# StructuralNeurobiologyLab/SyConn

Measured on AMD Instinct MI355X. Metric: segmented Mvoxels/s (whole node), 128^3 EM tiles, higher is better.
Workload: dtype bf16; 1 GPU; BASELINE configs[1]: semseg_spine 3D U-Net on 128^3 uint8 tiles, 96 tiles per GPU per step in launch sets of 8 (sd_forward_labels_batch), random-init weights, HOST TO HOST: pinned host uint8 tiles -> H2D -> kernels -> pinned host uint8 labels (stored by the last kernel, no copy), 3 HIP streams, 2 buffer sets; tiles_per_launch_set=8, parallelism=tile-sharded x1, hip_streams_per_gpu=3, collective=none

## Files before the change

### syconn_amd/csrc/sd_kernels.hip

```cpp
#include "sd_internal.h"
#include "../../include/syconn_dense.h"
#include <algorithm>
#include <cstdlib>
#include <mutex>
#include <string>
#include <type_traits>
#include <utility>

#include "sd_device.h"

#include "sd_conv_mfma.h"


template <typename T, int KZ, typename IN, bool SPLIT = false>
__global__ __launch_bounds__(256) void k_conv_first(const FirstParams p) {
    constexpr int BZ = sd_bz(KZ), BY = sd_by(KZ), BX = SD_BX;
    constexpr int PZ = KZ / 2;
    constexpr int HZ = BZ + KZ - 1, HY = BY + 2, HX = BX + 2;
    constexpr int NH = HZ * HY * HX;
    constexpr int NTAP = KZ * 9;
    constexpr int NSTEP = (NTAP + 1) / 2;
    __shared__ float patch[NH];

    const int tid = threadIdx.x, lane = tid & 63, wave = tid >> 6;
// ... 153 lines not shown
            for (int e = 0; e < 4; ++e) acc[0][j][4 * q + e] = acc[1][j][4 * q + e] = bs[e];
        }

    __shared__ __attribute__((aligned(16))) float gtab[GN ? 2 * 1024 : 4];
    const float* gss = nullptr;
    if constexpr (GN) {
        const float* const g = reinterpret_cast<const float*>(reinterpret_cast<const char*>(p.gn) + blockIdx.z * p.tstride);
        for (int i = tid; i < 2 * p.Cs; i += 256) gtab[i] = g[i];
        __syncthreads();
        gss = gtab;
    }
    for (int c = 0; c < p.nchunk; ++c) {
        v8 xf[2], wf[2];
#pragma unroll
        for (int i = 0; i < 2; ++i) {
            v8 val = {};
            if (mv[i]) {
                const int sc = (SPLIT && c >= p.nchunk / 3) ? c - p.nchunk / 3 : c;
                val = *reinterpret_cast<const v8*>(src + ((size_t)sc * p.Ps + upconv_src_index(p, m[i])) * SD_CHUNK + (lane >> 5) * 8);
                if constexpr (GN) val = gn_apply8<T>(val, gss + c * SD_CHUNK + (lane >> 5) * 8, gss + p.Cs + c * SD_CHUNK + (lane >> 5) * 8, p.gn_relu);
            }
            xf[i] = val;
        }
#pragma unroll
        for (int j = 0; j < 2; ++j) wf[j] = *reinterpret_cast<const v8*>(wp + ((size_t)(c * 2 + j) * 64 + lane) * 8);
#pragma unroll
        for (int i = 0; i < 2; ++i)
#pragma unroll
            for (int j = 0; j < 2; ++j) acc[i][j] = Act<T>::mfma(wf[j], xf[i], acc[i][j]);
    }

    T* const dst = reinterpret_cast<T*>(reinterpret_cast<char*>(p.dst) + blockIdx.z * p.tstride);
    StoreGuard<T> sguard;
    const int H2 = p.Hd, W2 = p.Wd;
    const int half = lane >> 5;
#pragma unroll
    for (int i = 0; i < 2; ++i) {
        const unsigned mu = mv[i] ? (unsigned)m[i] : 0u;
        const unsigned xy = mu % (unsigned)(p.W * p.H), z = mu / (unsigned)(p.W * p.H), y = xy / (unsigned)p.W, x = xy - y * (unsigned)p.W;
#pragma unroll
        for (int j = 0; j < 2; ++j) {
            const int nbase = (nb * 2 + j) * 32;
#pragma unroll
            for (int qp = 0; qp < 2; ++qp) {
                unsigned d[2][2], dl[2][2];
#pragma unroll
                for (int h = 0; h < 2; ++h) {
                    const int q = 2 * qp + h;
                    float v[4];
#pragma unroll
                    for (int e = 0; e < 4; ++e) {
                        v[e] = acc[i][j][4 * q + e];
                        if constexpr (SPLIT) v[e] *= p.oscale;
                        if (p.relu) v[e] = fmaxf(v[e], 0.f);
                    }
                    if constexpr (SPLIT) {
                        split_pk(v[0], v[1], d[h][0], dl[h][0]);
                        split_pk(v[2], v[3], d[h][1], dl[h][1]);
                    } else {
                        d[h][0] = Act<T>::pack2(v[0], v[1]);
                        d[h][1] = Act<T>::pack2(v[2], v[3]);
                    }
                    sguard.see_signed(d[h][0]); sguard.see_signed(d[h][1]);
                }
                swap32(d[0][0], d[1][0]);
                swap32(d[0][1], d[1][1]);
                if constexpr (SPLIT) { swap32(dl[0][0], dl[1][0]); swap32(dl[0][1], dl[1][1]); }
                const int n8 = nbase + 8 * (2 * qp + half);
                if (mv[i] && n8 < p.ntot) {
                    const int tap = n8 / p.Cd, co = n8 - tap * p.Cd;
                    const int a = (p.kz == 2) ? (tap >> 2) : 0, b = (tap >> 1) & 1, cx = tap & 1;
                    const size_t vo = ((size_t)(z * p.kz + a) * H2 + (2 * y + b)) * W2 + (2 * x + cx);
                    typedef __attribute__((ext_vector_type(4))) unsigned u4;
                    *reinterpret_cast<u4*>(dst + ((size_t)(co >> 4) * p.Pd + vo) * SD_CHUNK + (co & 15)) = u4{d[0][0], d[0][1], d[1][0], d[1][1]};
                    if constexpr (SPLIT)
                        *reinterpret_cast<u4*>(dst + ((size_t)((co + p.Cd) >> 4) * p.Pd + vo) * SD_CHUNK + (co & 15)) = u4{dl[0][0], dl[0][1], dl[1][0], dl[1][1]};
                }
            }
        }
    }
    sguard.flush(p.ovf);
}

template <typename T, int NCH, int NTAB, bool WL, bool GN, bool SPLIT = false, int G = 1>
__global__ __launch_bounds__(256) void k_upconv_rows(const UpconvParams p) {
    constexpr int NX = SPLIT ? 2 * NCH : NCH;
    constexpr int NV = SPLIT ? 3 * NCH : NCH;
    static_assert(!(SPLIT && GN), "split plan: no deferred GroupNorm");
    static_assert(G == 1 || (WL && NTAB % (2 * G) == 0), "channel groups: LDS weights, whole tiles of each x-tap per group");
    using v8 = typename Act<T>::v8;
    using v4 = typename Act<T>::v4;
    typedef __attribute__((ext_vector_type(4))) unsigned u4;
    constexpr int CDR = NTAB * 16;
    constexpr int NTL = NTAB / G;
    constexpr int TPT = NTL / 2;
    constexpr int CD = NTL * 16;
    constexpr int ROW = 4 * CD;
    constexpr int PPV = ROW / 16;
    constexpr int SWM = (PPV % 8 == 0) ? 7 : (PPV % 4 == 0) ? 3 : (PPV % 2 == 0) ? 1 : 0;
    extern __shared__ __attribute__((aligned(16))) char smem[];
    const int tid = threadIdx.x, lane = tid & 63, wave = tid >> 6, half = lane >> 5, vl = lane & 31;
    char* const tile = smem + wave * (32 * ROW);
    const long M = (long)p.D * p.H * p.W;
    const T* const src = reinterpret_cast<const T*>(reinterpret_cast<const char*>(p.src) + blockIdx.z * p.tstride);
    const T* const wp = reinterpret_cast<const T*>(p.wpack);
    char* const dst = reinterpret_cast<char*>(p.dst) + blockIdx.z * p.tstride;
    const int H2 = p.Hd, W2 = p.Wd;
    StoreGuard<T> sguard;
    __shared__ __attribute__((aligned(16))) float gtab[GN ? 2 * NCH * SD_CHUNK : 4];
    const float* gss = nullptr;
    if constexpr (GN) {
        const float* const g = reinterpret_cast<const float*>(reinterpret_cast<const char*>(p.gn) + blockIdx.z * p.tstride);
        for (int i = tid; i < 2 * NCH * SD_CHUNK; i += 256) gtab[i] = g[i];
        __syncthreads();
        gss = gtab;
    }

    const char* const wlds = smem + 4 * 32 * ROW;
    const int a_wg = WL ? (int)blockIdx.y / G : 0;
    const int grp = G > 1 ? (int)blockIdx.y % G : 0;
    auto tile_of = [&](int ab, int jl) { return G == 1 ? ab * NTAB + jl : ab * NTAB + (jl / TPT) * (NTAB / 2) + grp * TPT + jl % TPT; };
    if constexpr (WL && G > 1) {
        for (int i = tid; i < NTL * NV * 64; i += 256) {
            const int piece = i >> 6, jl = piece / NV, c = piece - jl * NV, tl = tile_of(a_wg, jl);
            *reinterpret_cast<u4*>(smem + 4 * 32 * ROW + (size_t)i * 16) =
                *reinterpret_cast<const u4*>(reinterpret_cast<const char*>(wp) + ((((size_t)(tl >> 1) * NV + c) * 2 + (tl & 1)) * 64 + (i & 63)) * 16);
        }
        __syncthreads();
    } else if constexpr (WL) {
        const int first_blk = (a_wg * NTAB) >> 1, last_blk = (a_wg * NTAB + NTAB - 1) >> 1;
        const int nbytes = (last_blk - first_blk + 1) * NV * 2048;
        const char* const wsrc = reinterpret_cast<const char*>(wp) + (size_t)first_blk * NV * 2048;
        for (int o = tid * 16; o < nbytes; o += 256 * 16)
            *reinterpret_cast<u4*>(smem + 4 * 32 * ROW + o) = *reinterpret_cast<const u4*>(wsrc + o);
        __syncthreads();
    }
    for (long m0 = ((long)blockIdx.x * 4 + wave) * 32; m0 < M; m0 += WL ? (long)gridDim.x * 128 : M) {
    const long m = m0 + vl;
    const bool mv = m < M;
    const size_t sidx = mv ? upconv_src_index(p, m) : 0;
    v8 xf[NX];
#pragma unroll
    for (int c = 0; c < NX; ++c) {
        v8 val = {};
        if (mv) val = *reinterpret_cast<const v8*>(src + ((size_t)c * p.Ps + sidx) * SD_CHUNK + half * 8);
        xf[c] = val;
    }
    if constexpr (GN) {
#pragma unroll
        for (int c = 0; c < NCH; ++c) {
            if (mv) xf[c] = gn_apply8<T>(xf[c], gss + c * SD_CHUNK + half * 8, gss + p.Cs + c * SD_CHUNK + half * 8, p.gn_relu);
            asm volatile("" ::: "memory");
        }
    }
    const int ab0 = WL ? a_wg : 0, nab = WL ? ab0 + 1 : p.kz * 2;
#pragma unroll 1
    for (int ab = ab0; ab < nab; ++ab) {
        f32x16 acc[NTL];
#pragma unroll
        for (int j = 0; j < NTL; ++j)
#pragma unroll
            for (int q = 0; q < 4; ++q) {
                const f32x4 b = *reinterpret_cast<const f32x4*>(p.bias + 32 * tile_of(ab, j) + 8 * q + 4 * half);
#pragma unroll
                for (int e = 0; e < 4; ++e) acc[j][4 * q + e] = b[e];
            }
#pragma unroll
        for (int c = 0; c < NV; ++c) {
#pragma unroll
            for (int j = 0; j < NTL; ++j) {
                const int tl = ab * NTAB + j;
                v8 wf;
                if constexpr (WL && G > 1) {
                    wf = *reinterpret_cast<const v8*>(wlds + (((j * NV + c) * 64 + lane) * 16));
                } else if constexpr (WL) {
                    const int tloc = ab * NTAB + j - 2 * ((ab0 * NTAB) >> 1);
                    wf = *reinterpret_cast<const v8*>(wlds + ((((tloc >> 1) * NV + c) * 2 + (tloc & 1)) * 64 + lane) * 16);
                } else {
                    wf = *reinterpret_cast<const v8*>(wp + ((((size_t)(tl >> 1) * NV + c) * 2 + (tl & 1)) * 64 + lane) * 8);
                }
                acc[j] = Act<T>::mfma(wf, xf[(SPLIT && c >= NCH) ? c - NCH : c], acc[j]);
            }
        }
#pragma unroll
        for (int pass = 0; pass < (SPLIT ? 2 : 1); ++pass) {
#pragma unroll
        for (int j = 0; j < NTL; ++j) {
#pragma unroll
            for (int q = 0; q < 4; ++q) {
                v4 o;
#pragma unroll
                for (int e = 0; e < 4; ++e) {
                    float v = acc[j][4 * q + e];
                    if constexpr (SPLIT) v *= p.oscale;
                    if (p.relu) v = fmaxf(v, 0.f);
                    if constexpr (SPLIT) {
                        const T h = (T)v;
                        o[e] = pass == 0 ? h : (T)(v - (float)h);
                    } else {
                        o[e] = (T)v;
                    }
                }
                if (pass == 0) {
                    typedef __attribute__((ext_vector_type(2))) unsigned u2g;
                    const u2g ob = __builtin_bit_cast(u2g, o);
                    sguard.see_signed(ob.x); sguard.see_signed(ob.y);
                }
                const int pc = (4 * j + q) ^ (vl & SWM);
                *reinterpret_cast<v4*>(tile + vl * ROW + pc * 16 + half * 8) = o;
            }
        }
        const int a = (p.kz == 2) ? (ab >> 1) : 0, b = ab & 1;
        size_t ovv[2];
        bool okv[2];
#pragma unroll
        for (int e = 0; e < 2; ++e) {
            const long mm = m0 + (lane >> 2) + 16 * e;
            okv[e] = mm < M;
            const unsigned mu = (unsigned)(okv[e] ? mm : 0), xy = mu % (unsigned)(p.W * p.H), z = mu / (unsigned)(p.W * p.H);
            const unsigned y = xy / (unsigned)p.W, x = xy - y * (unsigned)p.W;
            ovv[e] = ((size_t)(z * p.kz + a) * H2 + (2 * y + b)) * W2 + 2 * x;
        }
#pragma unroll
        for (int it = 0; it < (32 * PPV) / 64; ++it) {
            const int u = it * 64 + lane;
            const int chunk = u >> 7, r = u & 127;
            const int v = r >> 2, tap = (r >> 1) & 1, hf = r & 1;
            const int piece = tap * (CD / 8) + chunk * 2 + hf;
            if (okv[it & 1]) {
                const size_t ov = ovv[it & 1] + tap;
                const u4 val = *reinterpret_cast<const u4*>(tile + v * ROW + ((piece ^ (v & SWM)) * 16));
                *reinterpret_cast<u4*>(dst + (((size_t)(grp * (CD / 16) + chunk + pass * (CDR / 16)) * p.Pd + ov) * SD_CHUNK + hf * 8) * sizeof(T)) = val;
            }
        }
        }
    }
    }
    sguard.flush(p.ovf);
}

__device__ __forceinline__ void decode_zyx(unsigned v, unsigned W, unsigned H, int& x, int& y, int& z) {
    const unsigned r = v / W, zz = r / H;
    x = (int)(v - r * W); y = (int)(r - zz * H); z = (int)zz;
}
template <typename T>
__global__ __launch_bounds__(256) void k_maxpool(const PoolParams p) {
    using v8 = typename Act<T>::v8;
    const int ng = p.C / 8;
    const long total = (long)p.Do * p.Ho * p.Wo * ng;
    const T* const src = reinterpret_cast<const T*>(reinterpret_cast<const char*>(p.src) + blockIdx.z * p.tstride);
    T* const dst = reinterpret_cast<T*>(reinterpret_cast<char*>(p.dst) + blockIdx.z * p.tstride);
    const long npv = (long)p.Do * p.Ho * p.Wo;
    for (long idx = (long)blockIdx.x * 256 + threadIdx.x; idx < total; idx += (long)gridDim.x * 256) {
        const unsigned pv = (unsigned)(idx >> 1), ch = pv / (unsigned)npv;
        const long v = pv - ch * (unsigned)npv;
        const int cg = (int)ch * 2 + (int)(idx & 1);
        int xo, yo, zo;
        decode_zyx((unsigned)v, (unsigned)p.Wo, (unsigned)p.Ho, xo, yo, zo);
        float mx[8];
#pragma unroll
        for (int e = 0; e < 8; ++e) mx[e] = -INFINITY;
        for (int dz = 0; dz < p.kz; ++dz) {
            const int z = zo * p.kz + dz;
            if (z >= p.D) continue;
#pragma unroll
            for (int dy = 0; dy < 2; ++dy) {
                const int y = yo * 2 + dy;
                if (y >= p.H) continue;
#pragma unroll
                for (int dx = 0; dx < 2; ++dx) {
                    const int x = xo * 2 + dx;
                    if (x >= p.W) continue;
                    const v8 val = *reinterpret_cast<const v8*>(src + ((size_t)(cg >> 1) * p.Ps + ((size_t)z * p.H + y) * p.W + x) * SD_CHUNK + (cg & 1) * 8);
#pragma unroll
                    for (int e = 0; e < 8; ++e) mx[e] = fmaxf(mx[e], (float)val[e]);
                }
            }
        }
        v8 o;
#pragma unroll
        for (int e = 0; e < 8; ++e) o[e] = (T)mx[e];
        *reinterpret_cast<v8*>(dst + ((size_t)(cg >> 1) * p.Pd + v) * SD_CHUNK + (cg & 1) * 8) = o;
    }
}

template <typename T>
__global__ __launch_bounds__(256) void k_final(const FinalParams p) {
    using v8 = typename Act<T>::v8;
    const T* const src = reinterpret_cast<const T*>(reinterpret_cast<const char*>(p.src) + blockIdx.z * p.tstride);
    const float* __restrict__ w = p.w;
    for (long v = (long)blockIdx.x * 256 + threadIdx.x; v < p.nvox; v += (long)gridDim.x * 256) {
        float acc[8];
#pragma unroll
        for (int co = 0; co < 8; ++co) acc[co] = 0.f;
        const float* const gss = p.gn_scale_shift
            ? reinterpret_cast<const float*>(reinterpret_cast<const char*>(p.gn_scale_shift) + blockIdx.z * p.tstride) : nullptr;
        const int nc8 = p.Cs / 8;
        for (int g0 = 0; g0 < nc8; g0 += 8) {
            v8 xr[8];
#pragma unroll
            for (int k = 0; k < 8; ++k) {
                const int c8 = g0 + k;
                if (c8 < nc8)
                    xr[k] = *reinterpret_cast<const v8*>(src + ((size_t)(c8 >> 1) * p.nvox + v) * SD_CHUNK + (c8 & 1) * 8);
            }
#pragma unroll
            for (int k = 0; k < 8; ++k) {
                const int c8 = g0 + k;
                if (c8 >= nc8) break;
                if (gss) xr[k] = gn_apply8<T>(xr[k], gss + c8 * 8, gss + p.Cs + c8 * 8, p.gn_relu);
#pragma unroll
                for (int e = 0; e < 8; ++e) {
                    const float xf = (float)xr[k][e];
#pragma unroll
                    for (int co = 0; co < 8; ++co) acc[co] = fmaf(xf, w[co * p.Cs + c8 * 8 + e], acc[co]);
// ... 420 lines not shown
        return launch_conv_k<T, KZ, NT, 4, 0, 2, 2>(p, NB, s);
    }
    if (big) {
        const char* const cap_env = getenv("SD_WRES_CAP_KB");
        const size_t wres_cap = (size_t)(cap_env ? atoi(cap_env) : ((long)p.D * p.H * p.W >= (1l << 20) ? 150 : 96)) * 1024;
        if (conv_lds_bytes<KZ, NT, 8, 2, 2>(nstages, p.final_wfrag != nullptr) <= wres_cap) return launch_conv_k<T, KZ, NT, 8, 2>(p, NB, s);
        if constexpr (KZ == 3 && NT == 2) {
            const bool mt2 = getenv("SD_MT2") != nullptr;
            const bool z_ok = getenv("SD_MT4_D_RULE") ? (p.D % 8 == 0 || p.D >= 96) : ((p.D + 7) / 8 * 8) * 100 <= ((p.D + 3) / 4 * 4) * 105;
            if (!mt2 && !p.final_wfrag && (vox / 1024) * NB >= 256 && z_ok)
                return launch_conv_k<T, KZ, NT, 8, 0, 4>(p, NB, s);
        }
        if constexpr (KZ == 1 && NT == 2) {
            const bool no_p4 = getenv("SD_NO_PLANAR4") != nullptr;
            if (!no_p4 && !p.final_wfrag && (p.H % 32 == 0 || p.H >= 128 || !getenv("SD_PLANAR4_H_RULE")) && (vox / 512) * NB >= 1024)
                return launch_conv_k<T, KZ, NT, 4, 0, 4>(p, NB, s);
        }
        if constexpr (KZ == 1 && NT == 3) {
            const bool no_ring = getenv("SD_NO_RING") != nullptr;
            if (!no_ring && nstages >= 3 && conv_lds_bytes<KZ, NT, 8, 2, -3>(nstages, p.final_wfrag != nullptr) <= (size_t)SD_LDS_BYTES)
                return launch_conv_k<T, KZ, NT, 8, -3>(p, NB, s);
        }
        return launch_conv_k<T, KZ, NT, 8, 0>(p, NB, s);
    }
    if (conv_lds_bytes<KZ, NT, 4, 2, 2>(nstages, p.final_wfrag != nullptr) <= 80 * 1024) return launch_conv_k<T, KZ, NT, 4, 2>(p, NB, s);
    return launch_conv_k<T, KZ, NT, 4, 0>(p, NB, s);
}
template <typename T>
static int launch_conv2_t(const ConvParams& p, int KZ, int NT, int NB, hipStream_t s) {
    if (KZ == 3 && NT == 3) return launch_conv_knt<T, 3, 3>(p, NB, s);
    if (KZ == 1 && NT == 3) return launch_conv_knt<T, 1, 3>(p, NB, s);
    if (KZ == 3 && NT == 2) return launch_conv_knt<T, 3, 2>(p, NB, s);
    if (KZ == 3 && NT == 1) return launch_conv_knt<T, 3, 1>(p, NB, s);
    if (KZ == 1 && NT == 2) return launch_conv_knt<T, 1, 2>(p, NB, s);
    if (KZ == 1 && NT == 1) return launch_conv_knt<T, 1, 1>(p, NB, s);
    return SD_ERR_INVALID;
}
int launch_conv(const ConvParams& p, int act_dtype, int KZ, int NT, int NB, hipStream_t s) {
    if (act_dtype == SD_F16X2) return launch_conv_split(p, KZ, NT, NB, s);
    return act_dtype == SD_BF16 ? launch_conv2_t<bf16_t>(p, KZ, NT, NB, s) : launch_conv2_t<f16_t>(p, KZ, NT, NB, s);
}

template <typename T, typename IN>
static int launch_first_t(const FirstParams& p, int KZ, hipStream_t s) {
    SD_NOTE_KERNEL(sizeof(IN) == 1 ? (p.wpack3 && KZ == 1 ? "k_conv_first<uint8 input, bf16 MFMA on the exact values>" : "k_conv_first<uint8 input, f32 MFMA chain>")
                                   : "k_conv_first<float32 input, f32 MFMA chain>");
    dim3 grid(p.nbx * p.nby * p.nbz, 1, p.batch), block(256);
    if (KZ == 3) hipLaunchKernelGGL((k_conv_first<T, 3, IN>), grid, block, 0, s, p);
    else if (KZ == 1) hipLaunchKernelGGL((k_conv_first<T, 1, IN>), grid, block, 0, s, p);
    else return SD_ERR_INVALID;
    return SD_LAUNCH_CHECK();
}
int launch_first(const FirstParams& p, int act_dtype, int in_dtype, int KZ, hipStream_t s) {
    if (act_dtype == SD_F16X2) {
        SD_NOTE_KERNEL("k_conv_first<split-fp16, f32 MFMA chain>");
        dim3 grid(p.nbx * p.nby * p.nbz, 1, p.batch), block(256);
        if (KZ == 3 && in_dtype == SD_U8) hipLaunchKernelGGL((k_conv_first<f16_t, 3, uint8_t, true>), grid, block, 0, s, p);
        else if (KZ == 3) hipLaunchKernelGGL((k_conv_first<f16_t, 3, float, true>), grid, block, 0, s, p);
        else if (KZ == 1 && in_dtype == SD_U8) hipLaunchKernelGGL((k_conv_first<f16_t, 1, uint8_t, true>), grid, block, 0, s, p);
        else if (KZ == 1) hipLaunchKernelGGL((k_conv_first<f16_t, 1, float, true>), grid, block, 0, s, p);
        else return SD_ERR_INVALID;
        return SD_LAUNCH_CHECK();
    }
    if (act_dtype == SD_BF16)
        return in_dtype == SD_U8 ? launch_first_t<bf16_t, uint8_t>(p, KZ, s) : launch_first_t<bf16_t, float>(p, KZ, s);
    return in_dtype == SD_U8 ? launch_first_t<f16_t, uint8_t>(p, KZ, s) : launch_first_t<f16_t, float>(p, KZ, s);
}

template <typename T, int NCH, int NTAB>
static int launch_upconv_rows(const UpconvParams& p, hipStream_t s) {
    { static const std::string name = "k_upconv_rows<NCH=" + std::to_string(NCH) + ",NTAB=" + std::to_string(NTAB) + ">"; SD_NOTE_KERNEL(name.c_str()); }
    const long M = (long)p.D * p.H * p.W;
    if (M >= (1l << 31)) return SD_ERR_INVALID;
    dim3 grid((unsigned)((M + 127) / 128), 1, p.batch), block(256);
    if (p.gn) hipLaunchKernelGGL((k_upconv_rows<T, NCH, NTAB, false, true>), grid, block, 4 * 32 * 64 * NTAB, s, p);
    else hipLaunchKernelGGL((k_upconv_rows<T, NCH, NTAB, false, false>), grid, block, 4 * 32 * 64 * NTAB, s, p);
    return SD_LAUNCH_CHECK();
}
template <typename T, int NCH, int NTAB>
static int launch_upconv_rows_wl(const UpconvParams& p, hipStream_t s) {
    { static const std::string name = "k_upconv_rows<NCH=" + std::to_string(NCH) + ",NTAB=" + std::to_string(NTAB) + ",LDS weights>"; SD_NOTE_KERNEL(name.c_str()); }
    const long M = (long)p.D * p.H * p.W;
    if (M >= (1l << 31)) return SD_ERR_INVALID;
    const size_t lds = 4 * 32 * 64 * NTAB + (size_t)(NTAB / 2 + 2 * (NTAB & 1)) * NCH * 2048;
    auto kern = p.gn ? k_upconv_rows<T, NCH, NTAB, true, true> : k_upconv_rows<T, NCH, NTAB, true, false>;
    {
        static std::mutex mu;
        static LaunchCache cache[2][SD_MAX_DEVICES];
        int dev = 0;
        if (hipGetDevice(&dev) != hipSuccess || dev < 0 || dev >= SD_MAX_DEVICES) return SD_ERR_HIP;
        std::lock_guard<std::mutex> lock(mu);
        LaunchCache& c = cache[p.gn ? 1 : 0][dev];
        if (lds > c.attr_set) {
            if (hipFuncSetAttribute(reinterpret_cast<const void*>(kern), hipFuncAttributeMaxDynamicSharedMemorySize, (int)lds) !=
                hipSuccess) return SD_ERR_HIP;
            c.attr_set = lds;
        }
    }
    const int per_cu = std::max(1, (int)(SD_LDS_BYTES / lds));
    const long want = std::max(1L, (long)SD_NUM_CU * per_cu * 2 / (2 * p.kz * p.batch));
    dim3 grid((unsigned)std::min((M + 127) / 128, want), 2 * p.kz, p.batch), block(256);
    hipLaunchKernelGGL(kern, grid, block, lds, s, p);
    return SD_LAUNCH_CHECK();
}
template <typename T, int NCH, int NTAB, int G>
static int launch_upconv_rows_wl_g(const UpconvParams& p, hipStream_t s) {
    { static const std::string name = "k_upconv_rows<NCH=" + std::to_string(NCH) + ",NTAB=" + std::to_string(NTAB) + ",LDS weights,G=" + std::to_string(G) + ">"; SD_NOTE_KERNEL(name.c_str()); }
    const long M = (long)p.D * p.H * p.W;
    if (M >= (1l << 31) || p.gn) return SD_ERR_INVALID;
    constexpr int NTL = NTAB / G;
    const size_t lds = (size_t)4 * 32 * (4 * NTL * 16) + (size_t)NTL * NCH * 1024;
    auto kern = k_upconv_rows<T, NCH, NTAB, true, false, false, G>;
    if (lds > (size_t)SD_LDS_BYTES) return SD_ERR_INVALID;
    if (hipFuncSetAttribute(reinterpret_cast<const void*>(kern), hipFuncAttributeMaxDynamicSharedMemorySize, (int)lds) != hipSuccess) return SD_ERR_HIP;
    const int per_cu = std::max(1, (int)(SD_LDS_BYTES / lds));
    const long want = std::max(1L, (long)SD_NUM_CU * per_cu * 2 / (2 * p.kz * G * p.batch));
    dim3 grid((unsigned)std::min((M + 127) / 128, want), 2 * p.kz * G, p.batch), block(256);
    hipLaunchKernelGGL(kern, grid, block, lds, s, p);
    return SD_LAUNCH_CHECK();
}
bool upconv_rows_kernel(int nchunk, int Cd) {
    static const bool no_wl = getenv("SD_NO_UPCONV_WL") != nullptr;
    return (nchunk == 4 && Cd == 32) || (nchunk == 3 && Cd == 32) || (nchunk == 2 && Cd == 16) || (nchunk == 8 && Cd == 64 && !no_wl) ||
           (nchunk == 6 && Cd == 48) || (nchunk == 12 && Cd == 96 && !no_wl);
}

template <typename T>
static int launch_upconv_t(const UpconvParams& p, int NB, hipStream_t s) {
    SD_NOTE_KERNEL("k_upconv_mfma");
    static const bool no_wl = getenv("SD_NO_UPCONV_WL") != nullptr;
    if (p.nchunk == 4 && p.Cd == 32) return (no_wl || getenv("SD_UPCONV32_NO_WL")) ? launch_upconv_rows<T, 4, 2>(p, s) : launch_upconv_rows_wl<T, 4, 2>(p, s);
    if (p.nchunk == 3 && p.Cd == 32) return launch_upconv_rows<T, 3, 2>(p, s);
    if (p.nchunk == 2 && p.Cd == 16) return launch_upconv_rows<T, 2, 1>(p, s);
    if (p.nchunk == 8 && p.Cd == 64 && !no_wl) return launch_upconv_rows_wl<T, 8, 4>(p, s);
    if (p.nchunk == 6 && p.Cd == 48) return no_wl ? launch_upconv_rows<T, 6, 3>(p, s) : launch_upconv_rows_wl<T, 6, 3>(p, s);
    if (p.nchunk == 12 && p.Cd == 96 && !no_wl) return launch_upconv_rows_wl<T, 12, 6>(p, s);
    const bool many = (long)p.D * p.H * p.W * p.batch >= 98304;
    if (p.nchunk == 16 && p.Cd == 128 && !p.gn && !no_wl && many && !getenv("SD_UPCONV128_MFMA")) return launch_upconv_rows_wl_g<T, 16, 8, 2>(p, s);
    if (p.nchunk == 24 && p.Cd == 192 && !p.gn && !no_wl && many && !getenv("SD_UPCONV192_MFMA")) return launch_upconv_rows_wl_g<T, 24, 12, 6>(p, s);
    const long M = (long)p.D * p.H * p.W;
    if (M >= (1l << 31)) return SD_ERR_INVALID;
    dim3 grid((unsigned)((M + 255) / 256), NB, p.batch), block(256);
    if (p.gn) hipLaunchKernelGGL((k_upconv_mfma<T, true>), grid, block, 0, s, p);
    else hipLaunchKernelGGL((k_upconv_mfma<T, false>), grid, block, 0, s, p);
    return SD_LAUNCH_CHECK();
}
int launch_upconv(const UpconvParams& p, int act_dtype, int NB, hipStream_t s) {
    if (act_dtype == SD_F16X2) {
        SD_NOTE_KERNEL(p.nchunk == 12 || p.nchunk == 24 || p.nchunk == 18 || p.nchunk == 36 || p.nchunk == 48 ? "k_upconv_rows<split-fp16> / k_upconv_mfma<split-fp16>" : "k_upconv_mfma<split-fp16>");
        const long M = (long)p.D * p.H * p.W;
        if (M >= (1l << 31) || p.gn) return SD_ERR_INVALID;
        static const bool no_rows = getenv("SD_SPLIT_NO_ROWS") != nullptr;
        if (!no_rows && p.nchunk == 12 && p.Cd == 32 && getenv("SD_SPLIT_ROWS32_NO_WL")) {
            dim3 grid((unsigned)((M + 127) / 128), 1, p.batch), block(256);
            hipLaunchKernelGGL((k_upconv_rows<f16_t, 4, 2, false, false, true>), grid, block, 4 * 32 * 64 * 2, s, p);
            return SD_LAUNCH_CHECK();
        }
        auto rows_wl = [&](auto kern, int NTAB, int NV) -> int {
            const size_t lds = (size_t)4 * 32 * 64 * NTAB + (size_t)(NTAB / 2 + 2 * (NTAB & 1)) * NV * 2048;
            if (lds > (size_t)SD_LDS_BYTES) return SD_ERR_INVALID;
            if (hipFuncSetAttribute(reinterpret_cast<const void*>(kern), hipFuncAttributeMaxDynamicSharedMemorySize, (int)lds) != hipSuccess)
                return SD_ERR_HIP;
            const int per_cu = std::max(1, (int)(SD_LDS_BYTES / lds));
            const long want = std::max(1L, (long)SD_NUM_CU * per_cu * 2 / (2 * p.kz * p.batch));
            dim3 grid((unsigned)std::min((M + 127) / 128, want), 2 * p.kz, p.batch), block(256);
            hipLaunchKernelGGL(kern, grid, block, lds, s, p);
            return SD_LAUNCH_CHECK();
        };
        if (!no_rows && p.nchunk == 12 && p.Cd == 32 && !getenv("SD_SPLIT_ROWS32_NO_WL"))
            return rows_wl(k_upconv_rows<f16_t, 4, 2, true, false, true>, 2, 12);
        if (!no_rows && p.nchunk == 48 && p.Cd == 128 && M * p.batch >= 98304 && !getenv("SD_SPLIT_UPCONV128_MFMA")) {
            auto kern = k_upconv_rows<f16_t, 16, 8, true, false, true, 4>;
            const size_t lds = (size_t)4 * 32 * 128 + (size_t)2 * 48 * 1024;
            if (hipFuncSetAttribute(reinterpret_cast<const void*>(kern), hipFuncAttributeMaxDynamicSharedMemorySize, (int)lds) != hipSuccess)
                return SD_ERR_HIP;
            const long want = std::max(1L, (long)SD_NUM_CU * 2 / (2 * p.kz * 4 * p.batch));
            dim3 grid((unsigned)std::min((M + 127) / 128, want), 2 * p.kz * 4, p.batch), block(256);
            hipLaunchKernelGGL(kern, grid, block, lds, s, p);
            return SD_LAUNCH_CHECK();
        }
        if (!no_rows && p.nchunk == 24 && p.Cd == 64) return rows_wl(k_upconv_rows<f16_t, 8, 4, true, false, true>, 4, 24);
        if (!no_rows && p.nchunk == 18 && p.Cd == 48) return rows_wl(k_upconv_rows<f16_t, 6, 3, true, false, true>, 3, 18);
        if (!no_rows && p.nchunk == 36 && p.Cd == 96 && !getenv("SD_SPLIT_NO_ROWS96") && !getenv("SD_SPLIT_ROWS96_L2")) {
            auto kern = k_upconv_rows<f16_t, 12, 6, true, false, true, 3>;
            const size_t lds = (size_t)4 * 32 * 128 + (size_t)2 * 36 * 1024;
            if (hipFuncSetAttribute(reinterpret_cast<const void*>(kern), hipFuncAttributeMaxDynamicSharedMemorySize, (int)lds) != hipSuccess)
                return SD_ERR_HIP;
            const int per_cu = std::max(1, (int)(SD_LDS_BYTES / lds));
            const long want = std::max(1L, (long)SD_NUM_CU * per_cu * 2 / (2 * p.kz * 3 * p.batch));
            dim3 grid((unsigned)std::min((M + 127) / 128, want), 2 * p.kz * 3, p.batch), block(256);
            hipLaunchKernelGGL(kern, grid, block, lds, s, p);
            return SD_LAUNCH_CHECK();
        }
        if (!no_rows && p.nchunk == 36 && p.Cd == 96 && !getenv("SD_SPLIT_NO_ROWS96")) {
            auto kern = k_upconv_rows<f16_t, 12, 6, false, false, true>;
            const size_t lds = (size_t)4 * 32 * 64 * 6;
            if (hipFuncSetAttribute(reinterpret_cast<const void*>(kern), hipFuncAttributeMaxDynamicSharedMemorySize, (int)lds) != hipSuccess)
                return SD_ERR_HIP;
            dim3 grid((unsigned)((M + 127) / 128), 1, p.batch), block(256);
            hipLaunchKernelGGL(kern, grid, block, lds, s, p);
            return SD_LAUNCH_CHECK();
        }
        dim3 grid((unsigned)((M + 255) / 256), NB, p.batch), block(256);
        hipLaunchKernelGGL((k_upconv_mfma<f16_t, false, true>), grid, block, 0, s, p);
        return SD_LAUNCH_CHECK();
    }
    if (!getenv("SD_UPCONV_OLD") || p.gn)
        return act_dtype == SD_BF16 ? launch_upconv_t<bf16_t>(p, NB, s) : launch_upconv_t<f16_t>(p, NB, s);
    const long M = (long)p.D * p.H * p.W;
    dim3 grid((unsigned)((M + 255) / 256), NB, p.batch), block(256);
    if (act_dtype == SD_BF16) hipLaunchKernelGGL((k_upconv_mfma<bf16_t, false>), grid, block, 0, s, p);
    else hipLaunchKernelGGL((k_upconv_mfma<f16_t, false>), grid, block, 0, s, p);
    return SD_LAUNCH_CHECK();
}

int launch_pool(const PoolParams& p, int act_dtype, hipStream_t s) {
    SD_NOTE_KERNEL(act_dtype == SD_F16X2 ? "k_maxpool_split" : "k_maxpool");
    if (act_dtype == SD_F16X2) return launch_pool_split(p, s);
    const long total = (long)p.Do * p.Ho * p.Wo * (p.C / 8);
    if (total >= (1l << 32)) return SD_ERR_INVALID;
    dim3 grid(grid_for(total), 1, p.batch), block(256);
    if (act_dtype == SD_BF16) hipLaunchKernelGGL((k_maxpool<bf16_t>), grid, block, 0, s, p);
    else hipLaunchKernelGGL((k_maxpool<f16_t>), grid, block, 0, s, p);
    return SD_LAUNCH_CHECK();
}

int launch_final(const FinalParams& p, int act_dtype, hipStream_t s) {
    SD_NOTE_KERNEL(act_dtype == SD_F16X2 ? "k_final_split" : "k_final_mfma / k_final");
    if (act_dtype == SD_F16X2) return launch_final_split(p, s);
    static const bool scalar_final = getenv("SD_FINAL_SCALAR") != nullptr;
    const size_t lds = (size_t)(p.Cs / SD_CHUNK) * 2048 + (size_t)(2 * p.Cs + 8) * 4;
    if (p.wfrag && !scalar_final && lds <= 64 * 1024) {
        dim3 grid(grid_for(p.nvox, 256, 256 * 8), 1, p.batch), block(256);
        if (act_dtype == SD_BF16) hipLaunchKernelGGL((k_final_mfma<bf16_t>), grid, block, lds, s, p);
        else hipLaunchKernelGGL((k_final_mfma<f16_t>), grid, block, lds, s, p);
        return SD_LAUNCH_CHECK();
    }
    dim3 grid(grid_for(p.nvox), 1, p.batch), block(256);
    if (act_dtype == SD_BF16) hipLaunchKernelGGL((k_final<bf16_t>), grid, block, 0, s, p);
    else hipLaunchKernelGGL((k_final<f16_t>), grid, block, 0, s, p);
    return SD_LAUNCH_CHECK();
}

int launch_gn_finalize(const GnParams& p, hipStream_t s) {
    hipLaunchKernelGGL(k_gn_finalize, dim3(1, 1, p.batch), dim3(256), 0, s, p);
    return SD_LAUNCH_CHECK();
}

int launch_groupnorm(const GnParams& p, int act_dtype, hipStream_t s) {
    SD_NOTE_KERNEL(p.skip_stats ? (p.skip_apply ? "k_gn_finalize" : "k_gn_finalize + k_gn_apply") : (p.skip_apply ? "k_gn_stats + k_gn_finalize" : "k_gn_stats + k_gn_finalize + k_gn_apply"));
    if (act_dtype == SD_F16X2) return launch_groupnorm_split(p, s);
    const int ng = p.C / 8;
    const long nvox = (long)p.D * p.H * p.W;
    if (nvox * ng >= (1l << 32)) return SD_ERR_INVALID;
    dim3 g1(grid_for(nvox, 256 * 16, 1024), p.C / SD_CHUNK, p.batch), b1(256);
    dim3 g3(grid_for(nvox * ng), 1, p.batch), b3(256);
    dim3 gp(grid_for((long)std::max(p.pD, 1) * std::max(p.pH, 1) * std::max(p.pW, 1) * ng), 1, p.batch);
    if (act_dtype == SD_BF16) {
        if (!p.skip_stats) hipLaunchKernelGGL((k_gn_stats<bf16_t>), g1, b1, 0, s, p);
        hipLaunchKernelGGL(k_gn_finalize, dim3(1, 1, p.batch), dim3(256), 0, s, p);
        if (p.skip_apply) {}
        else if (p.pool_dst) hipLaunchKernelGGL((k_gn_apply_pool<bf16_t>), gp, b3, 0, s, p);
        else hipLaunchKernelGGL((k_gn_apply<bf16_t>), g3, b3, 0, s, p);
    } else {
        if (!p.skip_stats) hipLaunchKernelGGL((k_gn_stats<f16_t>), g1, b1, 0, s, p);
        hipLaunchKernelGGL(k_gn_finalize, dim3(1, 1, p.batch), dim3(256), 0, s, p);
        if (p.skip_apply) {}
        else if (p.pool_dst) hipLaunchKernelGGL((k_gn_apply_pool<f16_t>), gp, b3, 0, s, p);
// ... 100 lines not shown
```

Baseline: 3008 Mvox/s.

## Software-pipeline activation loads in persistent upconv rows kernel and stage bias in LDS

In the persistent LDS-weight upconv rows kernel, the next iteration's input activations are now loaded into registers before the current MFMA and store phase runs, so global load latency overlaps compute. Bias values are copied into LDS once per block instead of being reread from global memory each iteration. Weight fragments for a channel are gathered before the MFMAs, and the output writeback is split into an LDS read phase and a global store phase. The extra register buffer raises VGPR pressure and the bias table adds LDS, so prefetch is enabled only for selected configurations.

```diff
diff --git a/syconn_amd/csrc/sd_kernels.hip b/syconn_amd/csrc/sd_kernels.hip
--- a/syconn_amd/csrc/sd_kernels.hip
+++ b/syconn_amd/csrc/sd_kernels.hip
@@ -259,12 +259,21 @@
     sguard.flush(p.ovf);
 }
 
-template <typename T, int NCH, int NTAB, bool WL, bool GN, bool SPLIT = false, int G = 1>
+template <int NCH, int NTAB, bool SPLIT = false, int G = 1>
+constexpr size_t upconv_rows_weight_bytes() {
+    return G > 1 ? (size_t)(NTAB / G) * (SPLIT ? 3 * NCH : NCH) * 1024 : (size_t)(NTAB / 2 + 2 * (NTAB & 1)) * (SPLIT ? 3 * NCH : NCH) * 2048;
+}
+template <int NCH, int NTAB, bool SPLIT = false, int G = 1>
+constexpr size_t upconv_rows_wl_lds() {
+    return (size_t)4 * 32 * 64 * (NTAB / G) + upconv_rows_weight_bytes<NCH, NTAB, SPLIT, G>() + (size_t)(NTAB / G) * 128;
+}
+template <typename T, int NCH, int NTAB, bool WL, bool GN, bool SPLIT = false, int G = 1, bool PF = WL>
 __global__ __launch_bounds__(256) void k_upconv_rows(const UpconvParams p) {
     constexpr int NX = SPLIT ? 2 * NCH : NCH;
     constexpr int NV = SPLIT ? 3 * NCH : NCH;
     static_assert(!(SPLIT && GN), "split plan: no deferred GroupNorm");
     static_assert(G == 1 || (WL && NTAB % (2 * G) == 0), "channel groups: LDS weights, whole tiles of each x-tap per group");
+    static_assert(WL || !PF, "the prefetch belongs to the persistent loop");
     using v8 = typename Act<T>::v8;
     using v4 = typename Act<T>::v4;
     typedef __attribute__((ext_vector_type(4))) unsigned u4;
@@ -275,6 +284,7 @@
     constexpr int ROW = 4 * CD;
     constexpr int PPV = ROW / 16;
     constexpr int SWM = (PPV % 8 == 0) ? 7 : (PPV % 4 == 0) ? 3 : (PPV % 2 == 0) ? 1 : 0;
+    constexpr int NIT = (32 * PPV) / 64;
     extern __shared__ __attribute__((aligned(16))) char smem[];
     const int tid = threadIdx.x, lane = tid & 63, wave = tid >> 6, half = lane >> 5, vl = lane & 31;
     char* const tile = smem + wave * (32 * ROW);
@@ -297,6 +307,11 @@
     const int a_wg = WL ? (int)blockIdx.y / G : 0;
     const int grp = G > 1 ? (int)blockIdx.y % G : 0;
     auto tile_of = [&](int ab, int jl) { return G == 1 ? ab * NTAB + jl : ab * NTAB + (jl / TPT) * (NTAB / 2) + grp * TPT + jl % TPT; };
+    const float* const blds = reinterpret_cast<const float*>(wlds + upconv_rows_weight_bytes<NCH, NTAB, SPLIT, G>());
+    if constexpr (WL) {
+        for (int i = tid; i < NTL * 32; i += 256)
+            reinterpret_cast<float*>(smem + 4 * 32 * ROW + upconv_rows_weight_bytes<NCH, NTAB, SPLIT, G>())[i] = p.bias[32 * tile_of(a_wg, i >> 5) + (i & 31)];
+    }
     if constexpr (WL && G > 1) {
         for (int i = tid; i < NTL * NV * 64; i += 256) {
             const int piece = i >> 6, jl = piece / NV, c = piece - jl * NV, tl = tile_of(a_wg, jl);
@@ -312,17 +327,28 @@
             *reinterpret_cast<u4*>(smem + 4 * 32 * ROW + o) = *reinterpret_cast<const u4*>(wsrc + o);
         __syncthreads();
     }
-    for (long m0 = ((long)blockIdx.x * 4 + wave) * 32; m0 < M; m0 += WL ? (long)gridDim.x * 128 : M) {
-    const long m = m0 + vl;
-    const bool mv = m < M;
-    const size_t sidx = mv ? upconv_src_index(p, m) : 0;
+    auto load_x = [&](long mg, v8 (&x)[NX]) {
+        const long m = mg + vl;
+#pragma unroll
+        for (int c = 0; c < NX; ++c) x[c] = v8{};
+        if (m < M) {
+            const size_t sidx = upconv_src_index(p, m);
+#pragma unroll
+            for (int c = 0; c < NX; ++c) x[c] = *reinterpret_cast<const v8*>(src + ((size_t)c * p.Ps + sidx) * SD_CHUNK + half * 8);
+        }
+    };
+    const long mstep = WL ? (long)gridDim.x * 128 : M;
+    long m0 = ((long)blockIdx.x * 4 + wave) * 32;
     v8 xf[NX];
-#pragma unroll
-    for (int c = 0; c < NX; ++c) {
-        v8 val = {};
-        if (mv) val = *reinterpret_cast<const v8*>(src + ((size_t)c * p.Ps + sidx) * SD_CHUNK + half * 8);
-        xf[c] = val;
-    }
+    if constexpr (PF) {
+        load_x(m0, xf);
+        __builtin_amdgcn_s_waitcnt(0x0F70);
+    }
+    for (; m0 < M; m0 += mstep) {
+    v8 xn[PF ? NX : 1];
+    if constexpr (PF) load_x(m0 + mstep, xn);
+    else load_x(m0, xf);
+    const bool mv = m0 + vl < M;
     if constexpr (GN) {
 #pragma unroll
         for (int c = 0; c < NCH; ++c) {
@@ -338,26 +364,31 @@
         for (int j = 0; j < NTL; ++j)
 #pragma unroll
             for (int q = 0; q < 4; ++q) {
-                const f32x4 b = *reinterpret_cast<const f32x4*>(p.bias + 32 * tile_of(ab, j) + 8 * q + 4 * half);
+                const f32x4 b = WL ? *reinterpret_cast<const f32x4*>(blds + 32 * j + 8 * q + 4 * half)
+                                   : *reinterpret_cast<const f32x4*>(p.bias + 32 * tile_of(ab, j) + 8 * q + 4 * half);
 #pragma unroll
                 for (int e = 0; e < 4; ++e) acc[j][4 * q + e] = b[e];
             }
-#pragma unroll
-        for (int c = 0; c < NV; ++c) {
+        auto load_w = [&](int c, v8 (&wf)[NTL]) {
 #pragma unroll
             for (int j = 0; j < NTL; ++j) {
                 const int tl = ab * NTAB + j;
-                v8 wf;
                 if constexpr (WL && G > 1) {
-                    wf = *reinterpret_cast<const v8*>(wlds + (((j * NV + c) * 64 + lane) * 16));
+                    wf[j] = *reinterpret_cast<const v8*>(wlds + (((j * NV + c) * 64 + lane) * 16));
                 } else if constexpr (WL) {
                     const int tloc = ab * NTAB + j - 2 * ((ab0 * NTAB) >> 1);
-                    wf = *reinterpret_cast<const v8*>(wlds + ((((tloc >> 1) * NV + c) * 2 + (tloc & 1)) * 64 + lane) * 16);
+                    wf[j] = *reinterpret_cast<const v8*>(wlds + ((((tloc >> 1) * NV + c) * 2 + (tloc & 1)) * 64 + lane) * 16);
                 } else {
-                    wf = *reinterpret_cast<const v8*>(wp + ((((size_t)(tl >> 1) * NV + c) * 2 + (tl & 1)) * 64 + lane) * 8);
+                    wf[j] = *reinterpret_cast<const v8*>(wp + ((((size_t)(tl >> 1) * NV + c) * 2 + (tl & 1)) * 64 + lane) * 8);
                 }
-                acc[j] = Act<T>::mfma(wf, xf[(SPLIT && c >= NCH) ? c - NCH : c], acc[j]);
-            }
+            }
+        };
+#pragma unroll
+        for (int c = 0; c < NV; ++c) {
+            v8 wf[NTL];
+            load_w(c, wf);
+#pragma unroll
+            for (int j = 0; j < NTL; ++j) acc[j] = Act<T>::mfma(wf[j], xf[(SPLIT && c >= NCH) ? c - NCH : c], acc[j]);
         }
 #pragma unroll
         for (int pass = 0; pass < (SPLIT ? 2 : 1); ++pass) {
@@ -398,16 +429,36 @@
             const unsigned y = xy / (unsigned)p.W, x = xy - y * (unsigned)p.W;
             ovv[e] = ((size_t)(z * p.kz + a) * H2 + (2 * y + b)) * W2 + 2 * x;
         }
-#pragma unroll
-        for (int it = 0; it < (32 * PPV) / 64; ++it) {
+        u4 val[NIT];
+#pragma unroll
+        for (int it = 0; it < NIT; ++it) {
             const int u = it * 64 + lane;
             const int chunk = u >> 7, r = u & 127;
             const int v = r >> 2, tap = (r >> 1) & 1, hf = r & 1;
             const int piece = tap * (CD / 8) + chunk * 2 + hf;
-            if (okv[it & 1]) {
-                const size_t ov = ovv[it & 1] + tap;
-                const u4 val = *reinterpret_cast<const u4*>(tile + v * ROW + ((piece ^ (v & SWM)) * 16));
-                *reinterpret_cast<u4*>(dst + (((size_t)(grp * (CD / 16) + chunk + pass * (CDR / 16)) * p.Pd + ov) * SD_CHUNK + hf * 8) * sizeof(T)) = val;
+            val[it] = *reinterpret_cast<const u4*>(tile + v * ROW + ((piece ^ (v & SWM)) * 16));
+        }
+        if constexpr (PF) {
+            if (pass == (SPLIT ? 1 : 0)) {
+#pragma unroll
+                for (int c = 0; c < NX; ++c) {
+                    u4 t = __builtin_bit_cast(u4, xn[c]);
+                    asm volatile("" : "+v"(t));
+                    xf[c] = __builtin_bit_cast(v8, t);
+                }
+            }
+        }
+#pragma unroll
+        for (int e = 0; e < 2; ++e) {
+            if (okv[e]) {
+#pragma unroll
+                for (int it = e; it < NIT; it += 2) {
+                    const int u = it * 64 + lane;
+                    const int chunk = u >> 7, r = u & 127;
+                    const int tap = (r >> 1) & 1, hf = r & 1;
+                    const size_t ov = ovv[e] + tap;
+                    *reinterpret_cast<u4*>(dst + (((size_t)(grp * (CD / 16) + chunk + pass * (CDR / 16)) * p.Pd + ov) * SD_CHUNK + hf * 8) * sizeof(T)) = val[it];
+                }
             }
         }
         }
@@ -994,7 +1045,7 @@
     { static const std::string name = "k_upconv_rows<NCH=" + std::to_string(NCH) + ",NTAB=" + std::to_string(NTAB) + ",LDS weights>"; SD_NOTE_KERNEL(name.c_str()); }
     const long M = (long)p.D * p.H * p.W;
     if (M >= (1l << 31)) return SD_ERR_INVALID;
-    const size_t lds = 4 * 32 * 64 * NTAB + (size_t)(NTAB / 2 + 2 * (NTAB & 1)) * NCH * 2048;
+    const size_t lds = upconv_rows_wl_lds<NCH, NTAB>();
     auto kern = p.gn ? k_upconv_rows<T, NCH, NTAB, true, true> : k_upconv_rows<T, NCH, NTAB, true, false>;
     {
         static std::mutex mu;
@@ -1020,9 +1071,9 @@
     { static const std::string name = "k_upconv_rows<NCH=" + std::to_string(NCH) + ",NTAB=" + std::to_string(NTAB) + ",LDS weights,G=" + std::to_string(G) + ">"; SD_NOTE_KERNEL(name.c_str()); }
     const long M = (long)p.D * p.H * p.W;
     if (M >= (1l << 31) || p.gn) return SD_ERR_INVALID;
-    constexpr int NTL = NTAB / G;
-    const size_t lds = (size_t)4 * 32 * (4 * NTL * 16) + (size_t)NTL * NCH * 1024;
-    auto kern = k_upconv_rows<T, NCH, NTAB, true, false, false, G>;
+    const size_t lds = upconv_rows_wl_lds<NCH, NTAB, false, G>();
+    constexpr bool PF = upconv_rows_wl_lds<NCH, NTAB, false, G>() > (size_t)SD_LDS_BYTES / 2 || NCH <= 16;
+    auto kern = k_upconv_rows<T, NCH, NTAB, true, false, false, G, PF>;
     if (lds > (size_t)SD_LDS_BYTES) return SD_ERR_INVALID;
     if (hipFuncSetAttribute(reinterpret_cast<const void*>(kern), hipFuncAttributeMaxDynamicSharedMemorySize, (int)lds) != hipSuccess) return SD_ERR_HIP;
     const int per_cu = std::max(1, (int)(SD_LDS_BYTES / lds));
@@ -1068,8 +1119,7 @@
             hipLaunchKernelGGL((k_upconv_rows<f16_t, 4, 2, false, false, true>), grid, block, 4 * 32 * 64 * 2, s, p);
             return SD_LAUNCH_CHECK();
         }
-        auto rows_wl = [&](auto kern, int NTAB, int NV) -> int {
-            const size_t lds = (size_t)4 * 32 * 64 * NTAB + (size_t)(NTAB / 2 + 2 * (NTAB & 1)) * NV * 2048;
+        auto rows_wl = [&](auto kern, size_t lds) -> int {
             if (lds > (size_t)SD_LDS_BYTES) return SD_ERR_INVALID;
             if (hipFuncSetAttribute(reinterpret_cast<const void*>(kern), hipFuncAttributeMaxDynamicSharedMemorySize, (int)lds) != hipSuccess)
                 return SD_ERR_HIP;
@@ -1080,10 +1130,10 @@
             return SD_LAUNCH_CHECK();
         };
         if (!no_rows && p.nchunk == 12 && p.Cd == 32 && !getenv("SD_SPLIT_ROWS32_NO_WL"))
-            return rows_wl(k_upconv_rows<f16_t, 4, 2, true, false, true>, 2, 12);
+            return rows_wl(k_upconv_rows<f16_t, 4, 2, true, false, true, 1, false>, upconv_rows_wl_lds<4, 2, true>());
         if (!no_rows && p.nchunk == 48 && p.Cd == 128 && M * p.batch >= 98304 && !getenv("SD_SPLIT_UPCONV128_MFMA")) {
             auto kern = k_upconv_rows<f16_t, 16, 8, true, false, true, 4>;
-            const size_t lds = (size_t)4 * 32 * 128 + (size_t)2 * 48 * 1024;
+            const size_t lds = upconv_rows_wl_lds<16, 8, true, 4>();
             if (hipFuncSetAttribute(reinterpret_cast<const void*>(kern), hipFuncAttributeMaxDynamicSharedMemorySize, (int)lds) != hipSuccess)
                 return SD_ERR_HIP;
             const long want = std::max(1L, (long)SD_NUM_CU * 2 / (2 * p.kz * 4 * p.batch));
@@ -1091,11 +1141,11 @@
             hipLaunchKernelGGL(kern, grid, block, lds, s, p);
             return SD_LAUNCH_CHECK();
         }
-        if (!no_rows && p.nchunk == 24 && p.Cd == 64) return rows_wl(k_upconv_rows<f16_t, 8, 4, true, false, true>, 4, 24);
-        if (!no_rows && p.nchunk == 18 && p.Cd == 48) return rows_wl(k_upconv_rows<f16_t, 6, 3, true, false, true>, 3, 18);
+        if (!no_rows && p.nchunk == 24 && p.Cd == 64) return rows_wl(k_upconv_rows<f16_t, 8, 4, true, false, true>, upconv_rows_wl_lds<8, 4, true>());
+        if (!no_rows && p.nchunk == 18 && p.Cd == 48) return rows_wl(k_upconv_rows<f16_t, 6, 3, true, false, true>, upconv_rows_wl_lds<6, 3, true>());
         if (!no_rows && p.nchunk == 36 && p.Cd == 96 && !getenv("SD_SPLIT_NO_ROWS96") && !getenv("SD_SPLIT_ROWS96_L2")) {
             auto kern = k_upconv_rows<f16_t, 12, 6, true, false, true, 3>;
-            const size_t lds = (size_t)4 * 32 * 128 + (size_t)2 * 36 * 1024;
+            const size_t lds = upconv_rows_wl_lds<12, 6, true, 3>();
             if (hipFuncSetAttribute(reinterpret_cast<const void*>(kern), hipFuncAttributeMaxDynamicSharedMemorySize, (int)lds) != hipSuccess)
                 return SD_ERR_HIP;
             const int per_cu = std::max(1, (int)(SD_LDS_BYTES / lds));
```

Result: no change. 3031 Mvox/s, median of 6 (+0.8%).
